# bglid/GTCRN-Micro

Hardware: AMD Instinct MI355X
Metric: 16 kHz frames/sec (STFT->mask->iSTFT) (higher is better)
Workload: dtype f32; 1 GPU; offline wave->wave, B=256 clips/GPU x 4 s @16 kHz (T=251 frames), fp32, shipped checkpoint weights; batch_per_gpu=256, parallelism=1 independent utterance shards, no data-path collective

## Files before the change

### gtcrn_micro_amd/csrc/api.cpp

```cpp
#include "../../include/gtcrn_micro_hip.h"

#include <hip/hip_runtime.h>

#include <cmath>
#include <cstdint>
#include <cstdio>
#include <cstring>
#include <mutex>
#include <string>
#include <vector>

#include "kernels.h"
#include "layout.h"
#include "pack.h"

namespace {

thread_local std::string g_err;

int fail(int code, const std::string& msg) {
    g_err = msg;
    return code;
}
int hip_fail(hipError_t e, const char* what) {
// ... 32 lines not shown
    float* d_pfq = nullptr;
    int* d_pi = nullptr;
    float* d_twid = nullptr;
    int* d_pref = nullptr;
    bool var_spans = true;
    int stream_form = 0;
    std::vector<int> h_pi;
    long cap_bt = 0;
    int last_B = 0, last_T = 0;
    float* d_en0 = nullptr;
    float* d_en[4] = {nullptr, nullptr, nullptr, nullptr};
    float* d_g1 = nullptr;
    float* d_g2 = nullptr;
    float* d_spec_a = nullptr;
    float* d_spec_b = nullptr;
    float* d_rate_a = nullptr;
    float* d_rate_b = nullptr;
    long cap_rate = 0;
    bool debug = false;
    bool debug_keep_fused = false;
    float* d_dbg = nullptr;
    long dbg_cap_bt = 0;
    unsigned long long* d_stamps = nullptr;
    int stamps_cap_b = 0;
    float** d_ptr8 = nullptr;
    bool last_quant = false;
    bool last_fused_stream = false;
    bool timing = false;
    int timing_only = -1;
    std::vector<Timing> timings;
    std::vector<Timing> ev_pool;
};

namespace {

void free_workspace(gtcrn_model* m) {
    float** bufs[] = {&m->d_en0, &m->d_en[0], &m->d_en[1], &m->d_en[2], &m->d_en[3], &m->d_g1, &m->d_g2,
                      &m->d_spec_a, &m->d_spec_b};
    for (float** p : bufs) {
        if (*p) (void)hipFree(*p);
        *p = nullptr;
    }
    m->cap_bt = 0;
}

int ensure_workspace(gtcrn_model* m, int B, int T, hipStream_t s) {
    const long bt = (long)B * T;
    if (bt > m->cap_bt) {
        hipStreamCaptureStatus cs = hipStreamCaptureStatusNone;
        if (hipStreamIsCapturing(s, &cs) == hipSuccess && cs != hipStreamCaptureStatusNone)
            return fail(GTCRN_ERR_STATE, "workspace too small during stream capture: call gtcrn_model_reserve first");
        HIP_TRY(hipDeviceSynchronize());
        free_workspace(m);
        HIP_TRY(hipMalloc(&m->d_en0, sizeof(float) * bt * 65 * 16));
        for (int i = 0; i < 4; ++i) HIP_TRY(hipMalloc(&m->d_en[i], sizeof(float) * bt * 528));
        HIP_TRY(hipMalloc(&m->d_g1, sizeof(float) * bt * 528));
        HIP_TRY(hipMalloc(&m->d_g2, sizeof(float) * bt * 528));
        HIP_TRY(hipMalloc(&m->d_spec_a, sizeof(float) * bt * 514));
        HIP_TRY(hipMalloc(&m->d_spec_b, sizeof(float) * bt * 514));
        m->cap_bt = bt;
    }
    if (m->debug && bt > m->dbg_cap_bt) {
        if (m->d_dbg) (void)hipFree(m->d_dbg);
        m->d_dbg = nullptr;
        HIP_TRY(hipMalloc(&m->d_dbg, sizeof(float) * bt * (3 * 528 + 65 * 16 + 2 * 129)));
        m->dbg_cap_bt = bt;
    }
    if (m->debug && B + 2048 > m->stamps_cap_b) {
        const int rows = B + 2048;
        if (m->d_stamps) (void)hipFree(m->d_stamps);
        m->d_stamps = nullptr;
        HIP_TRY(hipMalloc(&m->d_stamps, sizeof(unsigned long long) * 4 * rows * 16));
        HIP_TRY(hipMemset(m->d_stamps, 0, sizeof(unsigned long long) * 4 * rows * 16));
        m->stamps_cap_b = rows;
// ... 24 lines not shown
    void end() {
        if (!on) return;
        (void)hipEventRecord(m->timings.back().b, s);
    }
};

static bool stream_wide_pays(int B) {
    constexpr double WIDE_COST = 1.5;
    const int ws = gtk::stream_wide_streams();
    const long r4 = ((B + 3) / 4 + 255) / 256, r7 = ((B + ws - 1) / ws + 255) / 256;
    return (double)r7 * WIDE_COST < (double)r4;
}

int run_model(gtcrn_model* m, const float* spec_in, long isb, long isf, long ist, float* spec_out, long osb, long osf,
              long ost, int B, int T, float* state, hipStream_t s, const int* lens = nullptr,
              const gtk::Quant* q = nullptr, bool front_done = false) {
    Timer tm(m, s);
    const float* pf = q ? m->d_pfq : m->d_pf;
    const bool offline = !state;
    m->last_quant = q != nullptr;
    m->last_fused_stream = false;
    if (state && T == 1 && !q && (!m->debug || m->debug_keep_fused) && m->stream_form != 1 && gtk::stream_ms_usable(isb, osb)) {
        const bool wide = m->stream_form == 3 || (m->stream_form == 0 && stream_wide_pays(B));
        unsigned long long* stamps = (m->debug && m->d_stamps) ? m->d_stamps : nullptr;
        tm.begin(wide ? K_STREAM_WIDE : K_STREAM_MS);
        if (wide) LAUNCH_TRY(gtk::launch_stream_wide(spec_in, isb, isf, spec_out, osb, osf, B, pf, m->d_pi, state, stamps, s));
        else LAUNCH_TRY(gtk::launch_stream_ms(spec_in, isb, isf, spec_out, osb, osf, B, pf, m->d_pi, state, stamps, s));
        tm.end();
        m->last_fused_stream = true;
        m->last_B = B;
        m->last_T = T;
// ... 30 lines not shown
            LAUNCH_TRY(gtk::launch_gtcn(m->d_en[3], m->d_g1, pf + gtl::P_GTCN, B, T, state, gtk::ST_G1_H, nullptr,
                                        stp ? stp + sst : nullptr, s));
        tm.end();
        tm.begin(K_GTCN2);
        if (!state)
            LAUNCH_TRY(gtk::launch_gtcn_band(m->d_g1, m->d_g2, pf + gtl::P_GTCN + gtl::GTCN_SIZE, B, T, lens, m->d_en[3], s,
                                             q, pref));
        else
            LAUNCH_TRY(gtk::launch_gtcn(m->d_g1, m->d_g2, pf + gtl::P_GTCN + gtl::GTCN_SIZE, B, T, state, gtk::ST_G2_H,
                                        m->d_en[3], stp ? stp + 2 * sst : nullptr, s));
        tm.end();
    }
    tm.begin(K_DECODER);
    LAUNCH_TRY(gtk::launch_decoder(m->d_g2, m->d_en0, m->d_en[0], m->d_en[1], m->d_en[2], m->d_en[3], spec_in, isb, isf,
                                   ist, spec_out, osb, osf, ost, B, T, lens, pf, m->d_pi, state,
                                   m->debug && !q ? m->d_dbg : nullptr, stp ? stp + 3 * sst : nullptr, s, q, pref));
    tm.end();
    m->last_B = B;
    m->last_T = T;
    return 0;
}

int check_model(gtcrn_model* m) {
    if (!m || !m->d_pf) return fail(GTCRN_ERR_STATE, "invalid model handle");
    HIP_TRY(hipSetDevice(m->device));
    return 0;
}

int upload_params(gtcrn_model* m, const float* h_params, long n) {
    std::vector<float> F(gtl::P_FLOATS);
    std::vector<int> I(gtl::P_INTS);
// ... 230 lines not shown
    int rc = check_model(m);
    if (rc) return rc;
    if (!d_wave || !d_wave_out || !d_win) return fail(GTCRN_ERR_ARG, "null pointer");
    if (B < 1) return fail(GTCRN_ERR_ARG, "B must be >= 1");
    if (L < 257) return fail(GTCRN_ERR_ARG, "reflect padding needs L > 256 samples");
    hipStream_t s = (hipStream_t)stream;
    const int T = (int)gtcrn_num_frames(L);
    rc = ensure_workspace(m, B, T, s);
    if (rc) return rc;
    const long sb = (long)T * 514, sf = 2, st = 514;
    Timer tm(m, s);
    tm.begin(K_FRONT);
    LAUNCH_TRY(gtk::launch_front(d_wave, L, nullptr, 0, 0, 0, B, T, d_lengths, d_win, m->d_twid, q ? m->d_pfq : m->d_pf,
                                 m->d_pi, m->d_spec_a, m->d_en0, m->d_en[0], s, q));
    tm.end();
    rc = run_model(m, m->d_spec_a, sb, sf, st, m->d_spec_b, sb, sf, st, B, T, nullptr, s, d_lengths, q, true);
    if (rc) return rc;
    tm.begin(K_ISTFT);
    LAUNCH_TRY(gtk::launch_istft(m->d_spec_b, sb, sf, st, B, T, d_lengths, d_win, m->d_twid, d_wave_out, s));
    tm.end();
    return 0;
}

int gtcrn_forward_wave(gtcrn_model* m, const float* d_wave, float* d_wave_out, int B, long L, const float* d_win,
                       void* stream) {
    return forward_wave_impl(m, d_wave, d_wave_out, B, L, nullptr, d_win, stream);
}

int gtcrn_forward_wave_var(gtcrn_model* m, const float* d_wave, float* d_wave_out, int B, long Lmax,
                           const int* d_lengths, const float* d_win, void* stream) {
// ... 868 lines not shown
```

### gtcrn_micro_amd/csrc/kernels.h

```cpp
#pragma once
#include <hip/hip_runtime.h>

namespace gtk {

constexpr int TC = 16;
constexpr int NW = 11;
constexpr int NTHR = NW * 64;
constexpr int NT2 = TC * 33 / 16;
constexpr int TPW = NT2 / NW;
constexpr int SHORT_T = (NW * 16) / 33;
constexpr int SHORT_T2 = (2 * NW * 16) / 33;
static_assert(TC * 33 % 16 == 0, "chunk must be a whole number of tiles");
static_assert(NT2 % NW == 0, "tiles must divide evenly over the waves");

constexpr int FRAMES_PER_WAVE = 2;
constexpr int ISTFT_BLOCKS = 7;

constexpr int WS_RING = 0;
constexpr int WS_TAIL = 512;
constexpr int WS_CNT = 768;
constexpr int WS_FLOATS = 772;
constexpr int WS_CNT_MAX = 1 << 30;
constexpr int WAVE_FRAMES = 2;
static_assert(WS_FLOATS % 4 == 0, "16-byte aligned rows");
// ... 6 lines not shown
constexpr int ST_DEC_H = ST_G2_H + 30 * 33 * 16;
constexpr int ST_DEC_E = ST_DEC_H + 3 * 2 * 33 * 16;
constexpr int ST_FLOATS = ST_DEC_E + 48;

struct Quant {
    float in_step = 0.f;
    float out_step = 0.f;
};

int configure_kernels();
int launch_stft(const float* wave, int B, long L, int T, const int* lens, const float* win, const float* twid,
                float* spec, long sb, long sf, long st, float* frames, hipStream_t s);
int launch_pcm16_convert(const void* src, void* dst, long n, int dir, hipStream_t s);
int launch_istft(const float* spec, long sb, long sf, long st, int B, int T, const int* lens, const float* win,
                 const float* twid, float* wave, hipStream_t s);
template <typename S>
int launch_wave_analysis(const S* in, long in_stride, int N, int nhops, int r, bool flush, const float* wstate,
                         const float* win, const float* twid, float* spec, hipStream_t s);
template <typename S>
int launch_wave_synthesis(const float* spec, const S* in, long in_stride, S* out, long out_stride, int N, int nhops, int r,
                          bool flush, float* wstate, const float* win, const float* twid, hipStream_t s);
constexpr int RS_THREADS = 256;
constexpr int RS_TILE = 1024;
constexpr int RS_SPAN = 3328;
constexpr int RS_LDS_TAPS = 1024;
constexpr int RATE_SPAN = 1024;
long resample_tile_span(int up, int down, int ntp);
template <typename SI, typename SO>
int launch_resample(const SI* in, long in_stride, const int* lens, long L, SO* out, long out_stride, int B, int up, int down,
                    int half, int ntp, const float* taps, hipStream_t s);
// ... 20 lines not shown
int launch_encoder(const float* spec, long sb, long sf, long st, int B, int T, const int* lens, const float* PF,
                   const int* PI, float* en0, float* en1, float* en2, float* en3, float* en4, float* state,
                   unsigned long long* stamps, hipStream_t s, const Quant* q = nullptr, bool front_done = false,
                   const int* pref = nullptr);
int launch_front(const float* wave, long L, const float* spec_in, long isb, long isf, long ist, int B, int T,
                 const int* lens, const float* win, const float* twid, const float* PF, const int* PI, float* spec_out,
                 float* en0, float* en1p, hipStream_t s, const Quant* q = nullptr);
int launch_gtcn(const float* xin, float* xout, const float* P, int B, int T, float* state, int st_off,
                const float* addend, unsigned long long* stamps, hipStream_t s);
int launch_gtcn_ms(const float* xin, float* xout1, float* xout2, const float* P, int B, float* state, hipStream_t s);
int launch_gtcn_band(const float* xin, float* xout, const float* P, int B, int T, const int* lens, const float* addend,
                     hipStream_t s, const Quant* q = nullptr, const int* pref = nullptr);
int launch_decoder(const float* xg, const float* en0, const float* en1, const float* en2, const float* en3,
                   const float* en4, const float* spec, long sb, long sf, long st, float* out, long osb, long osf,
                   long ost, int B, int T, const int* lens, const float* PF, const int* PI, float* state, float* dbg,
                   unsigned long long* stamps, hipStream_t s, const Quant* q = nullptr, const int* pref = nullptr);
bool var_spans_usable(int B);
int launch_len_prefix(const int* lens, int B, int T, int* pref, hipStream_t s);
int launch_stream_ms(const float* spec, long sb, long sf, float* out, long osb, long osf, int B, const float* PF,
                     const int* PI, float* state, unsigned long long* stamps, hipStream_t s);
int launch_stream_wide(const float* spec, long sb, long sf, float* out, long osb, long osf, int B, const float* PF,
                       const int* PI, float* state, unsigned long long* stamps, hipStream_t s);
int stream_wide_streams();
bool stream_ms_usable(long sb, long osb);
int launch_state_convert(float* state, int N, float* conv, float* tra, float* const* tcn8, const int* PI, int dir,
                         hipStream_t s);
int launch_conv2d_causal(const float* x, const float* cache, const float* w, const float* bias, float* y,
                         float* cache_out, int B, int Cin, int Cout, int T, int F, int kt, int kf, int dt, int df,
                         int pf, int groups, int transposed, int Fout, hipStream_t s);
int launch_selftest(const float* A, const float* Bm, const float* C, float* D, hipStream_t s);
int launch_selftest_split3(const float* x, long n, float* planes, float* joined, const float* A, const float* Bm,
// ... 4 lines not shown
```

### gtcrn_micro_amd/csrc/kernels.hip

```cpp
#include <hip/hip_runtime.h>

#include <cstdint>
#include <cstdio>
#include <cstdlib>
#include <type_traits>

#include "kernels.h"
#include "layout.h"

using namespace gtl;

namespace gtk {

typedef float f32x4 __attribute__((ext_vector_type(4)));
typedef float f32x2 __attribute__((ext_vector_type(2)));

__device__ __forceinline__ f32x4 ld4(const float* p) { return *reinterpret_cast<const f32x4*>(p); }
__device__ __forceinline__ void st4(float* p, f32x4 v) { *reinterpret_cast<f32x4*>(p) = v; }
__device__ __forceinline__ void copy_params(float* dst, const float* src, int n, int tid, int nthr) {
    for (int i = 4 * tid; i < n; i += 4 * nthr) st4(dst + i, ld4(src + i));
}
__device__ __forceinline__ f32x4 splat(float v) { f32x4 r = {v, v, v, v}; return r; }
__device__ __forceinline__ void lds_dma_1k(const float* gsrc_lane, const float* lds_piece) {
    const unsigned lds_dst = (unsigned)(size_t)(__attribute__((address_space(3))) const void*)lds_piece;
// ... 93 lines not shown
}
template <bool Q>
__device__ __forceinline__ float rq1(float v) {
    if constexpr (Q) return (float)(_Float16)v;
    else return v;
}
template <bool Q>
__device__ __forceinline__ f32x4 rq(const f32x4 v) {
    if constexpr (Q) {
        const h16x4 h = to_h4(v);
        f32x4 r = {(float)h[0], (float)h[1], (float)h[2], (float)h[3]};
        return r;
    } else {
        return v;
    }
}
template <bool Q>
__device__ __forceinline__ f32x4 mm1(const f32x4 A, const f32x4 b, f32x4 acc) {
    if constexpr (Q) {
        return mfma_h(to_h4(A), to_h4(b), acc);
    } else {
#pragma unroll
        for (int s = 0; s < 4; ++s) acc = mfma(A[s], b[s], acc);
        return acc;
    }
}
template <int N, bool Q = false>
__device__ __forceinline__ void mm16(const f32x4 A, const f32x4 (&x)[N], f32x4 (&acc)[N]) {
    if constexpr (Q) {
        const h16x4 ah = to_h4(A);
// ... 262 lines not shown
                    *ok = make_float2(old.x + ck * (ze.x + r.x), old.y + (k == 0 ? 0.f : ck * (ze.y + r.y)));
                    if (k == 0) { const float2 o2 = *on; *on = make_float2(o2.x + (zk.x - zk.y) * (1.0f / 512.0f), o2.y); }
                } else {
                    *ok = make_float2(ze.x + r.x, ze.y + r.y);
                    if (k == 0)
                        *on = make_float2(zk.x - zk.y, 0.f);
                }
            }
        }
        wave_lds_sync();
#pragma unroll
        for (int q = 0; q < 4; ++q) cur[q] = nxt[q];
    }
}

__global__ __launch_bounds__(FFT_WAVES * 64) void k_istft(const float* __restrict__ spec, long sb, long sf, long st,
                                                         int B, int T, const int* __restrict__ lens,
                                                         const float* __restrict__ win,
                                                         const float2* __restrict__ twid, float* __restrict__ wave) {
    __shared__ float2 s_tw[256];
    __shared__ float2 s_tw512[256];
    __shared__ float s_win[512];
    __shared__ float2 s_fa[ISTFT_BLOCKS + 1][256];
    __shared__ float2 s_fb[FFT_WAVES][256];
    float (*s_fr)[512] = reinterpret_cast<float (*)[512]>(&s_fa[0][0]);
    static_assert(ISTFT_BLOCKS + 1 <= 2 * FFT_WAVES, "one buffer per frame of the two rounds");
    const int tid = threadIdx.x, lane = tid & 63, wv = tid >> 6;
    for (int i = tid; i < 256; i += FFT_WAVES * 64) { s_tw[i] = twid[i]; s_tw512[i] = twid[256 + i]; }
    for (int i = tid; i < 512; i += FFT_WAVES * 64) s_win[i] = win[i];
    __syncthreads();
    const int groups = (T - 1 + ISTFT_BLOCKS - 1) / ISTFT_BLOCKS;
    const int b = blockIdx.x / groups, grp = blockIdx.x - b * groups;
    const int nblk = lens ? (lens[b] >> 8) : T - 1;
    const int j0 = grp * ISTFT_BLOCKS;
    if (j0 >= nblk) return;
    const int nfr = min(ISTFT_BLOCKS, nblk - j0) + 1;
    constexpr int ROUNDS = (ISTFT_BLOCKS + 1 + FFT_WAVES - 1) / FFT_WAVES;
    auto fetch = [&](int it, float2 (&vk)[4], float2 (&vm)[4]) {
        const int fi = it * FFT_WAVES + wv;
        const int t = j0 + (fi < nfr ? fi : 0);
        const float* x = spec + (long)b * sb + (long)t * st;
#pragma unroll
        for (int q = 0; q < 4; ++q) {
            const int k = lane + 64 * q;
            vk[q] = *reinterpret_cast<const float2*>(x + (long)k * sf);
            vm[q] = *reinterpret_cast<const float2*>(x + (long)(256 - k) * sf);
        }
    };
    float2 ck[4], cm[4], nk[4], nm[4];
    fetch(0, ck, cm);
    for (int it = 0; it < ROUNDS; ++it) {
        const int fi = it * FFT_WAVES + wv;
        const bool live = fi < nfr;
        float2* A = s_fa[fi < ISTFT_BLOCKS + 1 ? fi : ISTFT_BLOCKS];
        float2* Bf = s_fb[wv];
        if (it + 1 < ROUNDS) fetch(it + 1, nk, nm);
#pragma unroll
        for (int q = 0; q < 4; ++q) {
            const int k = lane + 64 * q;
            float2 xk = ck[q];
            float2 xm = cm[q];
            xm.y = -xm.y;
            if (k == 0) { xk.y = 0.f; xm.y = 0.f; }
            const float2 xe = make_float2(0.5f * (xk.x + xm.x), 0.5f * (xk.y + xm.y));
            float2 w = s_tw512[k];
            w.y = -w.y;
            const float2 xo = cmul(make_float2(0.5f * (xk.x - xm.x), 0.5f * (xk.y - xm.y)), w);
            A[k] = make_float2(xe.x - xo.y, xe.y + xo.x);
        }
        wave_lds_sync();
        fft256<1>(A, Bf, s_tw, lane);
        if (live) {
#pragma unroll
            for (int q = 0; q < 4; ++q) {
                const int m = lane + 64 * q;
                const float2 z = A[m];
                s_fr[fi][2 * m] = (z.x * (1.0f / 256.0f)) * s_win[2 * m];
                s_fr[fi][2 * m + 1] = (z.y * (1.0f / 256.0f)) * s_win[2 * m + 1];
            }
        }
        wave_lds_sync();
#pragma unroll
        for (int q = 0; q < 4; ++q) { ck[q] = nk[q]; cm[q] = nm[q]; }
    }
    __syncthreads();
    float* o = wave + (long)b * 256 * (T - 1);
    for (int idx = tid; idx < (nfr - 1) * 256; idx += FFT_WAVES * 64) {
        const int jb = idx >> 8, i = idx & 255;
        const float acc = s_fr[jb][256 + i] + s_fr[jb + 1][i];
        const float env = s_win[256 + i] * s_win[256 + i] + s_win[i] * s_win[i];
        o[(long)(j0 + jb) * 256 + i] = env > 1e-11f ? acc / env : acc;
    }
}

template <typename S>
__device__ __forceinline__ float wave_ld(const S* p) {
    if constexpr (std::is_same<S, short>::value) return (float)*p * (1.0f / 32768.0f);
    else return *p;
}
template <typename S>
__device__ __forceinline__ void wave_st(S* p, float y) {
    if constexpr (std::is_same<S, short>::value) *p = (short)(int)fminf(fmaxf(__builtin_rintf(y * 32768.0f), -32768.0f), 32767.0f);
    else *p = y;
}

template <typename S, bool FLUSH>
__global__ __launch_bounds__(FFT_WAVES * 64) void k_wave_analysis(const S* __restrict__ in, long in_stride, int N,
// ... 1772 lines not shown
    static constexpr int PT = MS ? 35 : 41;
    static constexpr int S = A + RWI * PT * RS;
    static constexpr int ZSZ = RW * DEC_Z_ROW * DEC_ZS;
    static constexpr int M = A + ZSZ;
    static constexpr int MSZ = (2 * RW * F0 + 4 + 3) & ~3;
    static constexpr int AEND = (S + RW * 33 * RSS) > (M + MSZ) ? (S + RW * 33 * RSS) : (M + MSZ);
    static constexpr int BS = AEND;
    static constexpr int FLOATS = BS + NBINS * 4;
    static_assert(M % 4 == 0 && BS % 4 == 0 && D_BS_W % 4 == 0 && D_BS_TAB % 4 == 0 && S % 4 == 0 && DL_SIZE % 4 == 0, "16B carve");
    static_assert(FLOATS * 4 <= 160 * 1024, "decoder LDS budget");
    static_assert(DEC_SIZE % 4 == 0 && I % 4 == 0 && H % 4 == 0 && A % 4 == 0 && E % 4 == 0, "16B carve");
};
constexpr int DEC_LDS_FLOATS = DecLds<TC, 1, false>::FLOATS;
constexpr int DEC_MS_LDS_FLOATS = DecLds<MS_ROWS, MS_STREAMS, true>::FLOATS;

template <bool DBG, int TPW, bool MS, bool Q, bool SPANS = false>
__global__ __launch_bounds__(NTHR) void k_decoder(const float* __restrict__ xg, const float* __restrict__ en0,
                                                 const float* __restrict__ en1, const float* __restrict__ en2,
                                                 const float* __restrict__ en3, const float* __restrict__ en4,
                                                 const float* __restrict__ spec, long sb, long sf, long st,
                                                 float* __restrict__ out, long osb, long osf, long ost, int T,
                                                 const int* __restrict__ lens, int NB, float qin, float qout,
                                                 const float* __restrict__ PF, const int* __restrict__ PI,
                                                 float* __restrict__ state, float* __restrict__ dbg,
                                                 unsigned long long* __restrict__ stamps) {
    extern __shared__ __attribute__((aligned(16))) float smem[];
    STAMP_INIT(SS)
    constexpr int RW = MS ? MS_ROWS : TC;
    constexpr int NS = MS ? MS_STREAMS : 1;
    using LD = DecLds<RW, NS, MS>;
    float* sP = smem + LD::P;
    int* sI = reinterpret_cast<int*>(smem + LD::I);
    float* sH = smem + LD::H;
    float* sEH = smem + LD::EH;
    int* sTB = reinterpret_cast<int*>(smem + LD::TB);
    float* sG = smem + LD::G;
    constexpr int RS = LD::RS;
    float* sW = smem + LD::A;
    float* sS = smem + LD::S;
    float* sZ = smem + LD::A;
    constexpr int ZS = DEC_ZS;
    float* sM = smem + LD::M;
    float* sBS = smem + LD::BS;
    const Lane L = lane_info();
    const int tid = L.tid, n = L.n, g = L.g;
    const int Tstride = T;
    static_assert(!SPANS || (!MS && !Q), "time spans: offline fp32 form");
    SpanIter sit;
    #ifdef GT_EXP_SAMEUTT
    int s_b = blockIdx.x & 7, s_fb = 0, s_wlo = 0, s_nT = T;
#else
    int s_b = blockIdx.x, s_fb = 0, s_wlo = 0, s_nT = T;
#endif
    if constexpr (SPANS) {
        if (!span_begin(sit, blockIdx.x, gridDim.x, NB, T, lens)) return;
        span_next(sit, NB, Tstride, lens, HALO_BLOCKS, s_b, s_fb, s_wlo, s_nT);
    }
    int b = s_b;
    constexpr bool SPLIT = !Q && kSplitDense;
    constexpr bool HALFW = Q && !MS;
    constexpr int DN_PIECES = SPLIT ? DN16_SIZE / 256 : (HALFW ? DN16_CHUNKS : 9);
    auto dense_fetch = [&](int j) {
// ... 2 lines not shown
        asm volatile("" : "+v"(lz));
        for (int pi = L.wave; pi < DN_PIECES; pi += NW) {
            const float* gsrc = src + pi * 256 + 4 * lz;
            const unsigned lds_dst = (unsigned)(size_t)(__attribute__((address_space(3))) void*)(sP + DL_DN + pi * 256);
            unsigned keep;
            asm volatile("s_mov_b32 %0, m0\n\ts_mov_b32 m0, %2\n\ts_nop 0\n\tglobal_load_lds_dwordx4 %1, off\n\ts_mov_b32 m0, %0"
                         : "=&s"(keep)
                         : "v"(gsrc), "s"(lds_dst)
                         : "memory");
        }
    };
    dense_fetch(0);
    constexpr bool SPLIT3 = SPLIT && kSplitDe3;
    copy_dec_params<SPLIT3>(sP, PF, tid, NTHR);
    if (tid < 48) sI[tid] = PI[I_DEC_BLK + tid];
    for (int f = tid; f < NBINS; f += NTHR) st4(sBS + f * 4, ld4(PF + P_DEC + D_BS_TAB + f * 4));
    if (tid < 4) sM[2 * RW * F0 + tid] = 0.f;
    float* stb = state ? state + (long)b * NS * ST_FLOATS : nullptr;
    const int nlive = MS ? min(NS, NB - b * NS) : 1;
    int tbase = 0;
    if constexpr (MS) {
        rings_load_ms<NS, SPLIT ? RS_WIDE : 16>(sH, sEH, stb, ST_DEC_H, ST_DEC_E, nlive, tid);
        if (tid < 8) sTB[tid] = tid < nlive ? reinterpret_cast<const int*>(stb + (long)tid * ST_FLOATS)[0] : 0;
    } else {
        tbase = stb ? reinterpret_cast<const int*>(stb)[0] : 0;
        rings_load(sH, sEH, stb ? stb + ST_DEC_H : nullptr, stb ? stb + ST_DEC_E : nullptr, tbase, tid);
    }
    const Tiles<TPW> tt = make_tiles<TPW>(L);
    wg_barrier_vm();

    const long nbt = MS ? (long)gridDim.x * T : (long)NB * T;
    const float* const spec0 = spec;
// ... 123 lines not shown
        for (int i = 0; i < TPW; ++i) {
            if (g < 3) {
                st4(sZ + (tt.tl[i] * DEC_Z_ROW + 1 + 2 * tt.ff[i]) * ZS + 4 * g, ze[i]);
                if (tt.ff[i] < 32) st4(sZ + (tt.tl[i] * DEC_Z_ROW + 2 + 2 * tt.ff[i]) * ZS + 4 * g, zo[i]);
            }
        }
        {
            int tz = tid;
            asm volatile("" : "+v"(tz));
            if (tz < RW * 2 * 4 && (tz & 3) < 3) {
                float z = 0.f;
                asm volatile("" : "+v"(z));
                st4(sZ + ((tz >> 3) * DEC_Z_ROW + ((tz >> 2) & 1) * (DEC_Z_ROW - 1)) * ZS + 4 * (tz & 3), splat(z));
            }
        }
        float2 spv[MASK_ITEMS];
        {
            int tz = tid;
            asm volatile("" : "+v"(tz));
            int tq, f;
            spec_item_first(tz, t_fast, tq, f);
            const float* sbase = spec + (long)t0 * st;
#pragma unroll
            for (int q = 0; q < MASK_ITEMS; ++q) {
                const bool ok = tq < nfr && f < NBINS;
                spv[q] = *reinterpret_cast<const float2*>(sbase + (ok ? f * sf32 + tq * st32 : 0));
                spec_item_next(t_fast, tq, f);
            }
        }
        STAMP(SS, 15)
        wg_barrier();
        STAMP(SS, 12)
// ... 4 lines not shown
            for (int i = 0; i < TPW; ++i) xn[i] = ldx<Q>(xgn + (unsigned)((tt.pp(i) < npn ? tt.pp(i) : 0) * 16 + 4 * g));
        }
        {
            static_assert(4 * F0 <= NTHR && RW % 2 == 0, "two threads per (o, f'')");
            int tz = tid;
            asm volatile("" : "+v"(tz));
            if (tz < 4 * F0) {
                const int h = tz >= 2 * F0 ? 1 : 0, c = tz - h * 2 * F0, o = c >= F0 ? 1 : 0, fq = c - o * F0;
                const int par = fq & 1, m = fq >> 1;
                const float* zr = sZ + (h * DEC_Z_ROW + 1 + m) * ZS;
                const float* r1 = zr + ZS + o * 5 + par;
                const float* r2 = zr + o * 5 + 2 + par;
                const float* r3 = zr - ZS + (par ? 10 : o * 5 + 4);
                const float bias = sP[dl(D_DE4_B) + o];
                float* mo = sM + (o * RW + h) * F0 + fq;
#pragma unroll
                for (int j = 0; j < RW / 2; ++j) {
                    constexpr int ZF = 2 * DEC_Z_ROW * ZS;
                    const float sum = bias + r1[j * ZF] + r2[j * ZF] + r3[j * ZF];
                    mo[j * 2 * F0] = rq1<Q>(fast_tanh(sum));
                }
            }
        }
        wg_barrier();
        STAMP(SS, 13)
        if (DBG)
            for (int idx = tid; idx < 2 * nfr * F0; idx += NTHR) {
                const int fq = idx % F0, ot = idx / F0, o = ot >= nfr ? 1 : 0, tq = ot - o * nfr;
                if (t0 + tq >= wlo)
                    dbg[3 * nbt * 528 + nbt * F1 * 16 + (((long)b * 2 + o) * Tstride + (ob - (long)b * Tstride) + t0 + tq) * F0 + fq] =
                        sM[(o * RW + tq) * F0 + fq];
            }
        {
            int tz = tid;
            asm volatile("" : "+v"(tz));
            int tq, f;
            spec_item_first(tz, t_fast, tq, f);
            float* obase = out + (long)t0 * ost;
            constexpr int GRP = 3;
            static_assert(MASK_ITEMS % GRP == 0, "mask items come in groups of three");
#pragma unroll
            for (int q0 = 0; q0 < MASK_ITEMS; q0 += GRP) {
                bool ok[GRP], wr[GRP];
                int fo[GRP];
                const float* m0[GRP];
                f32x4 tb[GRP];
#pragma unroll
                for (int j = 0; j < GRP; ++j) {
// ... 1 lines not shown
                    wr[j] = ok[j] && t0 + tq >= wlo;
                    const int fc = ok[j] ? f : 0, tc = ok[j] ? tq : 0;
                    tb[j] = ld4(sBS + fc * 4);
                    m0[j] = sM + tc * F0;
                    fo[j] = f * osf32 + tq * ost32;
                    spec_item_next(t_fast, tq, f);
                }
                float a0[GRP], a1[GRP], b0[GRP], b1[GRP];
#pragma unroll
                for (int j = 0; j < GRP; ++j) {
                    const float* mp = m0[j] + __float_as_int(tb[j][0]);
                    a0[j] = mp[0]; a1[j] = mp[1]; b0[j] = mp[RW * F0]; b1[j] = mp[RW * F0 + 1];
                }
#pragma unroll
                for (int j = 0; j < GRP; ++j) {
                    const bool two = tb[j][2] != 0.f;
                    const float mr = rq1<Q>(tb[j][1] * a0[j] + (two ? tb[j][2] * a1[j] : 0.f));
                    const float mi = rq1<Q>(tb[j][1] * b0[j] + (two ? tb[j][2] * b1[j] : 0.f));
                    float re = spv[q0 + j].x, im = spv[q0 + j].y;
                    if constexpr (Q) {
                        if (qin > 0.f) {
                            re = fminf(fmaxf(rintf(re / qin), -128.f), 127.f) * qin;
                            im = fminf(fmaxf(rintf(im / qin), -128.f), 127.f) * qin;
                        }
                        re = rq1<Q>(re);
                        im = rq1<Q>(im);
                    }
                    float yr = rq1<Q>(re * mr - im * mi), yi = rq1<Q>(im * mr + re * mi);
                    if constexpr (Q) {
                        if (qout > 0.f) {
                            yr = fminf(fmaxf(rintf(yr / qout), -128.f), 127.f) * qout;
                            yi = fminf(fmaxf(rintf(yi / qout), -128.f), 127.f) * qout;
                        }
                    }
                    if (wr[j]) *reinterpret_cast<float2*>(obase + fo[j]) = make_float2(yr, yi);
                }
            }
        }
        wg_barrier();
        STAMP(SS, 14)
    }
    if constexpr (SPANS) {
        if (span_next(sit, NB, Tstride, lens, HALO_BLOCKS, s_b, s_fb, s_wlo, s_nT)) {
// ... 3 lines not shown
            goto segment_top;
        }
    }
    STAMP_OUT(SS, stamps)
    if (stb) {
        wg_barrier();
        if constexpr (MS) {
            rings_store_ms<NS, SPLIT ? RS_WIDE : 16>(sH, sEH, stb, ST_DEC_H, ST_DEC_E, nlive, tid);
            if (tid < nlive) reinterpret_cast<int*>(stb + (long)tid * ST_FLOATS)[0] = (sTB[tid] + 1) & 0xFFFF;
        } else {
            rings_store(sH, sEH, stb + ST_DEC_H, stb + ST_DEC_E, tbase + T, tid);
            if (tid == 0) reinterpret_cast<int*>(stb)[0] = (tbase + T) & 0xFFFF;
        }
    }
}

__device__ __forceinline__ void stagger_start(int unit) {
#ifndef GT_EXP_NOSTAGGER
    if (unit > 0 && blockIdx.x < 256) {
        const int ph = ((blockIdx.x >> 3) + 32 * (blockIdx.x & 7)) & ((unit >> 8) - 1);
        for (int i = 0; i < ph * (unit & 255); ++i) __builtin_amdgcn_s_sleep(8);
    }
#endif
}
struct SmLds {
    static constexpr int RW = MS_ROWS, NS = MS_STREAMS;
    static constexpr int PE = 0;
    static constexpr int PG = PE + ENC_SIZE;
    static constexpr int PD = PG + 2 * GTCN_SIZE;
    static constexpr int I = PD + DL_SIZE;
// ... 1383 lines not shown
                       (const int*)nullptr, win,
                       reinterpret_cast<const float2*>(twid), gspec, sb, sf, st, (float*)nullptr);
    GT_LAUNCH_CHECK();
    return 0;
}

int launch_istft(const float* spec, long sb, long sf, long st, int B, int T, const int* lens, const float* win,
                 const float* twid, float* wave, hipStream_t s) {
    const int groups = (T - 1 + ISTFT_BLOCKS - 1) / ISTFT_BLOCKS;
    hipLaunchKernelGGL(k_istft, dim3(B * groups), dim3(FFT_WAVES * 64), 0, s, spec, sb, sf, st, B, T, lens, win,
                       reinterpret_cast<const float2*>(twid), wave);
    GT_LAUNCH_CHECK();
    return 0;
}

int configure_kernels() {
    hipError_t e;
    const void* enc[] = {reinterpret_cast<const void*>(k_encoder<TPW, false, false, false, true>),
                         reinterpret_cast<const void*>(k_encoder<TPW, false, false, true>),
                         reinterpret_cast<const void*>(k_encoder<1, false, false, true>),
                         reinterpret_cast<const void*>(k_encoder<2, false, false, true>),
                         reinterpret_cast<const void*>(k_encoder<TPW, false, false, false>),
                         reinterpret_cast<const void*>(k_encoder<1, false, false, false>),
                         reinterpret_cast<const void*>(k_encoder<2, false, false, false>),
                         reinterpret_cast<const void*>(k_encoder<TPW, false, true, false>)};
    const void* fr[] = {reinterpret_cast<const void*>(k_front<true, false>), reinterpret_cast<const void*>(k_front<false, false>),
                        reinterpret_cast<const void*>(k_front<true, true>), reinterpret_cast<const void*>(k_front<false, true>)};
    for (const void* f : fr) {
        e = hipFuncSetAttribute(f, hipFuncAttributeMaxDynamicSharedMemorySize, FR_LDS_FLOATS * 4);
        if (e != hipSuccess) return (int)e;
// ... 26 lines not shown
    if (e != hipSuccess) return (int)e;
    e = hipFuncSetAttribute(reinterpret_cast<const void*>(k_gtcn_band<true>), hipFuncAttributeMaxDynamicSharedMemorySize,
                            GB_LDS_FLOATS * 4);
    if (e != hipSuccess) return (int)e;
    e = hipFuncSetAttribute(reinterpret_cast<const void*>(k_gtcn_band<false, true>), hipFuncAttributeMaxDynamicSharedMemorySize,
                            GB_LDS_FLOATS * 4);
    if (e != hipSuccess) return (int)e;
    const void* dec[] = {reinterpret_cast<const void*>(k_decoder<false, TPW, false, false, true>),
                         reinterpret_cast<const void*>(k_decoder<true, TPW, false, false, true>),
                         reinterpret_cast<const void*>(k_decoder<false, TPW, false, false>),
                         reinterpret_cast<const void*>(k_decoder<true, TPW, false, false>),
                         reinterpret_cast<const void*>(k_decoder<false, 1, false, false>),
                         reinterpret_cast<const void*>(k_decoder<true, 1, false, false>),
                         reinterpret_cast<const void*>(k_decoder<false, 2, false, false>),
                         reinterpret_cast<const void*>(k_decoder<true, 2, false, false>),
                         reinterpret_cast<const void*>(k_decoder<false, TPW, false, true>)};
    for (const void* f : dec) {
        e = hipFuncSetAttribute(f, hipFuncAttributeMaxDynamicSharedMemorySize, DEC_LDS_FLOATS * 4);
        if (e != hipSuccess) return (int)e;
    }
    return 0;
}

static bool use_multi_stream(int T, const float* state, long sb) {
    return state != nullptr && T == 1 && (MS_ROWS - 1) * (sb < 0 ? -sb : sb) < (1L << 31);
}

int launch_front(const float* wave, long L, const float* spec_in, long isb, long isf, long ist, int B, int T,
                 const int* lens, const float* win, const float* twid, const float* PF, const int* PI, float* spec_out,
                 float* en0, float* en1p, hipStream_t s, const Quant* q) {
    const long wgs = ((long)B * T + FR_WAVES - 1) / FR_WAVES;
// ... 100 lines not shown
    if (pl.nA)
        hipLaunchKernelGGL(k_gtcn_band<false>, dim3(pl.nA), dim3(NTHR), GB_LDS_FLOATS * 4, s, xin, xout, P, pl.nA, T, lens,
                           addend);
    if (pl.nwgB) {
        const long o = (long)pl.nA * T * 528;
        hipLaunchKernelGGL((k_gtcn_band<false, true>), dim3(pl.nwgB), dim3(NTHR), GB_LDS_FLOATS * 4, s, xin + o, xout + o, P,
                           B - pl.nA, T, lens, addend ? addend + o : nullptr);
    }
    GT_LAUNCH_CHECK();
    return 0;
}

int launch_decoder(const float* xg, const float* en0, const float* en1, const float* en2, const float* en3,
                   const float* en4, const float* spec, long sb, long sf, long st, float* out, long osb, long osf,
                   long ost, int B, int T, const int* lens, const float* PF, const int* PI, float* state, float* dbg,
                   unsigned long long* stamps, hipStream_t s, const Quant* q, const int* pref) {
    if (pref && !state && !q) {
        const int nwg = var_span_workgroups(B);
        if (dbg)
            hipLaunchKernelGGL((k_decoder<true, TPW, false, false, true>), dim3(nwg), dim3(NTHR), DEC_LDS_FLOATS * 4, s, xg, en0,
                               en1, en2, en3, en4, spec, sb, sf, st, out, osb, osf, ost, T, pref, B, 0.f, 0.f, PF, PI, state, dbg,
                               stamps);
        else
            hipLaunchKernelGGL((k_decoder<false, TPW, false, false, true>), dim3(nwg), dim3(NTHR), DEC_LDS_FLOATS * 4, s, xg, en0,
                               en1, en2, en3, en4, spec, sb, sf, st, out, osb, osf, ost, T, pref, B, 0.f, 0.f, PF, PI, state, dbg,
                               stamps);
        GT_LAUNCH_CHECK();
        return 0;
    }
    SpanPlan pl = span_plan(B, T, HALO_BLOCKS, !state && !q && lens == nullptr);
    if (dbg && pl.nA && pl.nwgB) {
// ... 373 lines not shown
```

Baseline: 58.18 million frames/s.

## Hand off raw mask to iSTFT and apply band gain there

In the offline wave-to-wave path the decoder now writes only the raw tanh mask (258 floats per frame) to a new buffer, skipping the band-split gain and complex multiply on the spectrum. The iSTFT kernel reads the mask alongside the input spectrum, expands it through the band table in LDS and applies the complex ratio mask before the inverse FFT. The intent is to drop the decoder's spectrum read, its 514-float-per-frame masked spectrum write, and one decoder LDS barrier, at the cost of extra registers and LDS traffic in the iSTFT, now pinned to an occupancy of 5 waves per EU.

New measurement: 58.15 million frames/s. Within noise of the previous version (-0.1%).

```diff
diff --git a/gtcrn_micro_amd/csrc/api.cpp b/gtcrn_micro_amd/csrc/api.cpp
--- a/gtcrn_micro_amd/csrc/api.cpp
+++ b/gtcrn_micro_amd/csrc/api.cpp
@@ -70,6 +70,7 @@
     float* d_g2 = nullptr;
     float* d_spec_a = nullptr;
     float* d_spec_b = nullptr;
+    float* d_mask = nullptr;
     float* d_rate_a = nullptr;
     float* d_rate_b = nullptr;
     long cap_rate = 0;
@@ -92,7 +93,7 @@
 
 void free_workspace(gtcrn_model* m) {
     float** bufs[] = {&m->d_en0, &m->d_en[0], &m->d_en[1], &m->d_en[2], &m->d_en[3], &m->d_g1, &m->d_g2,
-                      &m->d_spec_a, &m->d_spec_b};
+                      &m->d_spec_a, &m->d_spec_b, &m->d_mask};
     for (float** p : bufs) {
         if (*p) (void)hipFree(*p);
         *p = nullptr;
@@ -114,6 +115,7 @@
         HIP_TRY(hipMalloc(&m->d_g2, sizeof(float) * bt * 528));
         HIP_TRY(hipMalloc(&m->d_spec_a, sizeof(float) * bt * 514));
         HIP_TRY(hipMalloc(&m->d_spec_b, sizeof(float) * bt * 514));
+        HIP_TRY(hipMalloc(&m->d_mask, sizeof(float) * bt * gtk::MASK_ROW));
         m->cap_bt = bt;
     }
     if (m->debug && bt > m->dbg_cap_bt) {
@@ -168,7 +170,7 @@
 
 int run_model(gtcrn_model* m, const float* spec_in, long isb, long isf, long ist, float* spec_out, long osb, long osf,
               long ost, int B, int T, float* state, hipStream_t s, const int* lens = nullptr,
-              const gtk::Quant* q = nullptr, bool front_done = false) {
+              const gtk::Quant* q = nullptr, bool front_done = false, bool mask_out = false) {
     Timer tm(m, s);
     const float* pf = q ? m->d_pfq : m->d_pf;
     const bool offline = !state;
@@ -229,7 +231,7 @@
     tm.begin(K_DECODER);
     LAUNCH_TRY(gtk::launch_decoder(m->d_g2, m->d_en0, m->d_en[0], m->d_en[1], m->d_en[2], m->d_en[3], spec_in, isb, isf,
                                    ist, spec_out, osb, osf, ost, B, T, lens, pf, m->d_pi, state,
-                                   m->debug && !q ? m->d_dbg : nullptr, stp ? stp + 3 * sst : nullptr, s, q, pref));
+                                   m->debug && !q ? m->d_dbg : nullptr, stp ? stp + 3 * sst : nullptr, s, q, pref, mask_out));
     tm.end();
     m->last_B = B;
     m->last_T = T;
@@ -490,6 +492,17 @@
     LAUNCH_TRY(gtk::launch_front(d_wave, L, nullptr, 0, 0, 0, B, T, d_lengths, d_win, m->d_twid, q ? m->d_pfq : m->d_pf,
                                  m->d_pi, m->d_spec_a, m->d_en0, m->d_en[0], s, q));
     tm.end();
+    const bool mask_out = gtk::mask_handoff_enabled() && !q && !m->debug;
+    if (mask_out) {
+        const long mr = gtk::MASK_ROW;
+        rc = run_model(m, m->d_spec_a, sb, sf, st, m->d_mask, (long)T * mr, 1, mr, B, T, nullptr, s, d_lengths, q, true, true);
+        if (rc) return rc;
+        tm.begin(K_ISTFT);
+        LAUNCH_TRY(gtk::launch_istft_mask(m->d_spec_a, sb, sf, st, m->d_mask, m->d_pf, B, T, d_lengths, d_win, m->d_twid,
+                                          d_wave_out, s));
+        tm.end();
+        return 0;
+    }
     rc = run_model(m, m->d_spec_a, sb, sf, st, m->d_spec_b, sb, sf, st, B, T, nullptr, s, d_lengths, q, true);
     if (rc) return rc;
     tm.begin(K_ISTFT);
diff --git a/gtcrn_micro_amd/csrc/kernels.h b/gtcrn_micro_amd/csrc/kernels.h
--- a/gtcrn_micro_amd/csrc/kernels.h
+++ b/gtcrn_micro_amd/csrc/kernels.h
@@ -44,6 +44,10 @@
 int launch_pcm16_convert(const void* src, void* dst, long n, int dir, hipStream_t s);
 int launch_istft(const float* spec, long sb, long sf, long st, int B, int T, const int* lens, const float* win,
                  const float* twid, float* wave, hipStream_t s);
+constexpr int MASK_ROW = 258;
+bool mask_handoff_enabled();
+int launch_istft_mask(const float* spec, long sb, long sf, long st, const float* mask, const float* PF, int B, int T,
+                      const int* lens, const float* win, const float* twid, float* wave, hipStream_t s);
 template <typename S>
 int launch_wave_analysis(const S* in, long in_stride, int N, int nhops, int r, bool flush, const float* wstate,
                          const float* win, const float* twid, float* spec, hipStream_t s);
@@ -94,7 +98,8 @@
 int launch_decoder(const float* xg, const float* en0, const float* en1, const float* en2, const float* en3,
                    const float* en4, const float* spec, long sb, long sf, long st, float* out, long osb, long osf,
                    long ost, int B, int T, const int* lens, const float* PF, const int* PI, float* state, float* dbg,
-                   unsigned long long* stamps, hipStream_t s, const Quant* q = nullptr, const int* pref = nullptr);
+                   unsigned long long* stamps, hipStream_t s, const Quant* q = nullptr, const int* pref = nullptr,
+                   bool mask_out = false);
 bool var_spans_usable(int B);
 int launch_len_prefix(const int* lens, int B, int T, int* pref, hipStream_t s);
 int launch_stream_ms(const float* spec, long sb, long sf, float* out, long osb, long osf, int B, const float* PF,
diff --git a/gtcrn_micro_amd/csrc/kernels.hip b/gtcrn_micro_amd/csrc/kernels.hip
--- a/gtcrn_micro_amd/csrc/kernels.hip
+++ b/gtcrn_micro_amd/csrc/kernels.hip
@@ -131,6 +131,17 @@
     } else {
         return v;
     }
+}
+template <bool Q>
+__device__ __forceinline__ void bs_gain(float w0, float w1, float a0, float a1, float b0, float b1, float& mr, float& mi) {
+    const bool two = w1 != 0.f;
+    mr = rq1<Q>(w0 * a0 + (two ? w1 * a1 : 0.f));
+    mi = rq1<Q>(w0 * b0 + (two ? w1 * b1 : 0.f));
+}
+template <bool Q>
+__device__ __forceinline__ void crm_apply(float re, float im, float mr, float mi, float& yr, float& yi) {
+    yr = rq1<Q>(re * mr - im * mi);
+    yi = rq1<Q>(im * mr + re * mi);
 }
 template <bool Q>
 __device__ __forceinline__ f32x4 mm1(const f32x4 A, const f32x4 b, f32x4 acc) {
@@ -423,10 +434,11 @@
     }
 }
 
-__global__ __launch_bounds__(FFT_WAVES * 64) void k_istft(const float* __restrict__ spec, long sb, long sf, long st,
-                                                         int B, int T, const int* __restrict__ lens,
-                                                         const float* __restrict__ win,
-                                                         const float2* __restrict__ twid, float* __restrict__ wave) {
+template <bool MIN>
+__device__ __forceinline__ void istft_body(const float* __restrict__ spec, long sb, long sf, long st, int B, int T,
+                                           const int* __restrict__ lens, const float* __restrict__ win,
+                                           const float2* __restrict__ twid, float* __restrict__ wave,
+                                           const float* __restrict__ mask, const float* __restrict__ bstab) {
     __shared__ float2 s_tw[256];
     __shared__ float2 s_tw512[256];
     __shared__ float s_win[512];
@@ -445,7 +457,8 @@
     if (j0 >= nblk) return;
     const int nfr = min(ISTFT_BLOCKS, nblk - j0) + 1;
     constexpr int ROUNDS = (ISTFT_BLOCKS + 1 + FFT_WAVES - 1) / FFT_WAVES;
-    auto fetch = [&](int it, float2 (&vk)[4], float2 (&vm)[4]) {
+    constexpr int NMR = MIN ? 5 : 1;
+    auto fetch = [&](int it, float2 (&vk)[4], float2 (&vm)[4], float (&vr)[NMR]) {
         const int fi = it * FFT_WAVES + wv;
         const int t = j0 + (fi < nfr ? fi : 0);
         const float* x = spec + (long)b * sb + (long)t * st;
@@ -455,15 +468,52 @@
             vk[q] = *reinterpret_cast<const float2*>(x + (long)k * sf);
             vm[q] = *reinterpret_cast<const float2*>(x + (long)(256 - k) * sf);
         }
+        if constexpr (MIN) {
+            const float* mrow = mask + ((long)b * T + t) * MASK_ROW;
+#pragma unroll
+            for (int q = 0; q < 4; ++q) vr[q] = mrow[lane + 64 * q];
+            vr[4] = mrow[256 + (lane & 1)];
+        }
     };
+    int bi[MIN ? 8 : 1];
+    float bw0[MIN ? 8 : 1], bw1[MIN ? 8 : 1];
+    if constexpr (MIN) {
+#pragma unroll
+        for (int q = 0; q < 8; ++q) {
+            const int f = q < 4 ? lane + 64 * q : 256 - (lane + 64 * (q - 4));
+            const f32x4 row = ld4(bstab + f * 4);
+            bi[q] = __float_as_int(row[0]); bw0[q] = row[1]; bw1[q] = row[2];
+        }
+    }
     float2 ck[4], cm[4], nk[4], nm[4];
-    fetch(0, ck, cm);
+    float cr[NMR], nr[NMR];
+    fetch(0, ck, cm, cr);
     for (int it = 0; it < ROUNDS; ++it) {
         const int fi = it * FFT_WAVES + wv;
         const bool live = fi < nfr;
         float2* A = s_fa[fi < ISTFT_BLOCKS + 1 ? fi : ISTFT_BLOCKS];
         float2* Bf = s_fb[wv];
-        if (it + 1 < ROUNDS) fetch(it + 1, nk, nm);
+        if (it + 1 < ROUNDS) fetch(it + 1, nk, nm, nr);
+        if constexpr (MIN) {
+            float* mb = reinterpret_cast<float*>(Bf);
+#pragma unroll
+            for (int q = 0; q < 4; ++q) mb[lane + 64 * q] = cr[q];
+            if (lane < 2) mb[256 + lane] = cr[4];
+            wave_lds_sync();
+            float a0[8], a1[8], b0[8], b1[8];
+#pragma unroll
+            for (int q = 0; q < 8; ++q) {
+                const float* mp = mb + bi[q];
+                a0[q] = mp[0]; a1[q] = mp[1]; b0[q] = mp[F0]; b1[q] = mp[F0 + 1];
+            }
+#pragma unroll
+            for (int q = 0; q < 8; ++q) {
+                float mr, mi;
+                bs_gain<false>(bw0[q], bw1[q], a0[q], a1[q], b0[q], b1[q], mr, mi);
+                float2& v = q < 4 ? ck[q] : cm[q - 4];
+                crm_apply<false>(v.x, v.y, mr, mi, v.x, v.y);
+            }
+        }
 #pragma unroll
         for (int q = 0; q < 4; ++q) {
             const int k = lane + 64 * q;
@@ -491,6 +541,8 @@
         wave_lds_sync();
 #pragma unroll
         for (int q = 0; q < 4; ++q) { ck[q] = nk[q]; cm[q] = nm[q]; }
+#pragma unroll
+        for (int q = 0; q < NMR; ++q) cr[q] = nr[q];
     }
     __syncthreads();
     float* o = wave + (long)b * 256 * (T - 1);
@@ -500,6 +552,20 @@
         const float env = s_win[256 + i] * s_win[256 + i] + s_win[i] * s_win[i];
         o[(long)(j0 + jb) * 256 + i] = env > 1e-11f ? acc / env : acc;
     }
+}
+__global__ __launch_bounds__(FFT_WAVES * 64) void k_istft(const float* __restrict__ spec, long sb, long sf, long st,
+                                                         int B, int T, const int* __restrict__ lens,
+                                                         const float* __restrict__ win,
+                                                         const float2* __restrict__ twid, float* __restrict__ wave) {
+    istft_body<false>(spec, sb, sf, st, B, T, lens, win, twid, wave, nullptr, nullptr);
+}
+__global__ __launch_bounds__(FFT_WAVES * 64) __attribute__((amdgpu_waves_per_eu(5, 5))) void k_istft_mask(const float* __restrict__ spec, long sb, long sf, long st,
+                                                              int B, int T, const int* __restrict__ lens,
+                                                              const float* __restrict__ win,
+                                                              const float2* __restrict__ twid, float* __restrict__ wave,
+                                                              const float* __restrict__ mask,
+                                                              const float* __restrict__ bstab) {
+    istft_body<true>(spec, sb, sf, st, B, T, lens, win, twid, wave, mask, bstab);
 }
 
 template <typename S>
@@ -2302,16 +2368,16 @@
 constexpr int DEC_LDS_FLOATS = DecLds<TC, 1, false>::FLOATS;
 constexpr int DEC_MS_LDS_FLOATS = DecLds<MS_ROWS, MS_STREAMS, true>::FLOATS;
 
-template <bool DBG, int TPW, bool MS, bool Q, bool SPANS = false>
-__global__ __launch_bounds__(NTHR) void k_decoder(const float* __restrict__ xg, const float* __restrict__ en0,
-                                                 const float* __restrict__ en1, const float* __restrict__ en2,
-                                                 const float* __restrict__ en3, const float* __restrict__ en4,
-                                                 const float* __restrict__ spec, long sb, long sf, long st,
-                                                 float* __restrict__ out, long osb, long osf, long ost, int T,
-                                                 const int* __restrict__ lens, int NB, float qin, float qout,
-                                                 const float* __restrict__ PF, const int* __restrict__ PI,
-                                                 float* __restrict__ state, float* __restrict__ dbg,
-                                                 unsigned long long* __restrict__ stamps) {
+template <bool DBG, int TPW, bool MS, bool Q, bool SPANS, bool MOUT>
+__device__ __forceinline__ void decoder_body(const float* __restrict__ xg, const float* __restrict__ en0,
+                                             const float* __restrict__ en1, const float* __restrict__ en2,
+                                             const float* __restrict__ en3, const float* __restrict__ en4,
+                                             const float* __restrict__ spec, long sb, long sf, long st,
+                                             float* __restrict__ out, long osb, long osf, long ost, int T,
+                                             const int* __restrict__ lens, int NB, float qin, float qout,
+                                             const float* __restrict__ PF, const int* __restrict__ PI,
+                                             float* __restrict__ state, float* __restrict__ dbg,
+                                             unsigned long long* __restrict__ stamps) {
     extern __shared__ __attribute__((aligned(16))) float smem[];
     STAMP_INIT(SS)
     constexpr int RW = MS ? MS_ROWS : TC;
@@ -2334,6 +2400,9 @@
     const int tid = L.tid, n = L.n, g = L.g;
     const int Tstride = T;
     static_assert(!SPANS || (!MS && !Q), "time spans: offline fp32 form");
+    static_assert(!MOUT || (!MS && !Q), "mask-out: offline fp32 form");
+    static_assert(MASK_ROW == 2 * F0, "mask hand-off row");
+    constexpr bool KEEP_M = !MOUT || DBG;
     SpanIter sit;
     #ifdef GT_EXP_SAMEUTT
     int s_b = blockIdx.x & 7, s_fb = 0, s_wlo = 0, s_nT = T;
@@ -2366,8 +2435,8 @@
     constexpr bool SPLIT3 = SPLIT && kSplitDe3;
     copy_dec_params<SPLIT3>(sP, PF, tid, NTHR);
     if (tid < 48) sI[tid] = PI[I_DEC_BLK + tid];
-    for (int f = tid; f < NBINS; f += NTHR) st4(sBS + f * 4, ld4(PF + P_DEC + D_BS_TAB + f * 4));
-    if (tid < 4) sM[2 * RW * F0 + tid] = 0.f;
+    if constexpr (!MOUT) for (int f = tid; f < NBINS; f += NTHR) st4(sBS + f * 4, ld4(PF + P_DEC + D_BS_TAB + f * 4));
+    if (KEEP_M && tid < 4) sM[2 * RW * F0 + tid] = 0.f;
     float* stb = state ? state + (long)b * NS * ST_FLOATS : nullptr;
     const int nlive = MS ? min(NS, NB - b * NS) : 1;
     int tbase = 0;
@@ -2521,8 +2590,8 @@
                 st4(sZ + ((tz >> 3) * DEC_Z_ROW + ((tz >> 2) & 1) * (DEC_Z_ROW - 1)) * ZS + 4 * (tz & 3), splat(z));
             }
         }
-        float2 spv[MASK_ITEMS];
-        {
+        float2 spv[MOUT ? 1 : MASK_ITEMS];
+        if constexpr (!MOUT) {
             int tz = tid;
             asm volatile("" : "+v"(tz));
             int tq, f;
@@ -2557,15 +2626,22 @@
                 const float* r3 = zr - ZS + (par ? 10 : o * 5 + 4);
                 const float bias = sP[dl(D_DE4_B) + o];
                 float* mo = sM + (o * RW + h) * F0 + fq;
+                float* mg = MOUT ? out + (long)t0 * ost : nullptr;
+                const int mgo = h * MASK_ROW + o * F0 + fq;
 #pragma unroll
                 for (int j = 0; j < RW / 2; ++j) {
                     constexpr int ZF = 2 * DEC_Z_ROW * ZS;
                     const float sum = bias + r1[j * ZF] + r2[j * ZF] + r3[j * ZF];
-                    mo[j * 2 * F0] = rq1<Q>(fast_tanh(sum));
+                    const float mv = rq1<Q>(fast_tanh(sum));
+                    if constexpr (KEEP_M) mo[j * 2 * F0] = mv;
+                    if constexpr (MOUT) {
+                        const int tq = h + 2 * j;
+                        if (tq < nfr && t0 + tq >= wlo) __builtin_nontemporal_store(mv, mg + mgo + j * 2 * MASK_ROW);
+                    }
                 }
             }
         }
-        wg_barrier();
+        if constexpr (KEEP_M) wg_barrier();
         STAMP(SS, 13)
         if (DBG)
             for (int idx = tid; idx < 2 * nfr * F0; idx += NTHR) {
@@ -2574,7 +2650,7 @@
                     dbg[3 * nbt * 528 + nbt * F1 * 16 + (((long)b * 2 + o) * Tstride + (ob - (long)b * Tstride) + t0 + tq) * F0 + fq] =
                         sM[(o * RW + tq) * F0 + fq];
             }
-        {
+        if constexpr (!MOUT) {
             int tz = tid;
             asm volatile("" : "+v"(tz));
             int tq, f;
@@ -2606,9 +2682,8 @@
                 }
 #pragma unroll
                 for (int j = 0; j < GRP; ++j) {
-                    const bool two = tb[j][2] != 0.f;
-                    const float mr = rq1<Q>(tb[j][1] * a0[j] + (two ? tb[j][2] * a1[j] : 0.f));
-                    const float mi = rq1<Q>(tb[j][1] * b0[j] + (two ? tb[j][2] * b1[j] : 0.f));
+                    float mr, mi;
+                    bs_gain<Q>(tb[j][1], tb[j][2], a0[j], a1[j], b0[j], b1[j], mr, mi);
                     float re = spv[q0 + j].x, im = spv[q0 + j].y;
                     if constexpr (Q) {
                         if (qin > 0.f) {
@@ -2618,7 +2693,8 @@
                         re = rq1<Q>(re);
                         im = rq1<Q>(im);
                     }
-                    float yr = rq1<Q>(re * mr - im * mi), yi = rq1<Q>(im * mr + re * mi);
+                    float yr, yi;
+                    crm_apply<Q>(re, im, mr, mi, yr, yi);
                     if constexpr (Q) {
                         if (qout > 0.f) {
                             yr = fminf(fmaxf(rintf(yr / qout), -128.f), 127.f) * qout;
@@ -2652,6 +2728,25 @@
         }
     }
 }
+#define GT_DEC_PARAMS                                                                                                 \
+    const float *__restrict__ xg, const float *__restrict__ en0, const float *__restrict__ en1,                      \
+        const float *__restrict__ en2, const float *__restrict__ en3, const float *__restrict__ en4,                 \
+        const float *__restrict__ spec, long sb, long sf, long st, float *__restrict__ out, long osb, long osf,      \
+        long ost, int T, const int *__restrict__ lens, int NB, float qin, float qout, const float *__restrict__ PF,  \
+        const int *__restrict__ PI, float *__restrict__ state, float *__restrict__ dbg,                              \
+        unsigned long long *__restrict__ stamps
+#define GT_DEC_ARGS                                                                                                   \
+    xg, en0, en1, en2, en3, en4, spec, sb, sf, st, out, osb, osf, ost, T, lens, NB, qin, qout, PF, PI, state, dbg, stamps
+template <bool DBG, int TPW, bool MS, bool Q, bool SPANS = false>
+__global__ __launch_bounds__(NTHR) void k_decoder(GT_DEC_PARAMS) {
+    decoder_body<DBG, TPW, MS, Q, SPANS, false>(GT_DEC_ARGS);
+}
+template <int TPW, bool SPANS>
+__global__ __launch_bounds__(NTHR) void k_decoder_mout(GT_DEC_PARAMS) {
+    decoder_body<false, TPW, false, false, SPANS, true>(GT_DEC_ARGS);
+}
+#undef GT_DEC_PARAMS
+#undef GT_DEC_ARGS
 
 __device__ __forceinline__ void stagger_start(int unit) {
 #ifndef GT_EXP_NOSTAGGER
@@ -4065,6 +4160,23 @@
     return 0;
 }
 
+bool mask_handoff_enabled() {
+#ifdef GT_MASK_IN_DECODER
+    return false;
+#else
+    return true;
+#endif
+}
+
+int launch_istft_mask(const float* spec, long sb, long sf, long st, const float* mask, const float* PF, int B, int T,
+                      const int* lens, const float* win, const float* twid, float* wave, hipStream_t s) {
+    const int groups = (T - 1 + ISTFT_BLOCKS - 1) / ISTFT_BLOCKS;
+    hipLaunchKernelGGL(k_istft_mask, dim3(B * groups), dim3(FFT_WAVES * 64), 0, s, spec, sb, sf, st, B, T, lens, win,
+                       reinterpret_cast<const float2*>(twid), wave, mask, PF + P_DEC + D_BS_TAB);
+    GT_LAUNCH_CHECK();
+    return 0;
+}
+
 int configure_kernels() {
     hipError_t e;
     const void* enc[] = {reinterpret_cast<const void*>(k_encoder<TPW, false, false, false, true>),
@@ -4121,7 +4233,11 @@
                          reinterpret_cast<const void*>(k_decoder<true, 1, false, false>),
                          reinterpret_cast<const void*>(k_decoder<false, 2, false, false>),
                          reinterpret_cast<const void*>(k_decoder<true, 2, false, false>),
-                         reinterpret_cast<const void*>(k_decoder<false, TPW, false, true>)};
+                         reinterpret_cast<const void*>(k_decoder<false, TPW, false, true>),
+                         reinterpret_cast<const void*>(k_decoder_mout<TPW, true>),
+                         reinterpret_cast<const void*>(k_decoder_mout<TPW, false>),
+                         reinterpret_cast<const void*>(k_decoder_mout<1, false>),
+                         reinterpret_cast<const void*>(k_decoder_mout<2, false>)};
     for (const void* f : dec) {
         e = hipFuncSetAttribute(f, hipFuncAttributeMaxDynamicSharedMemorySize, DEC_LDS_FLOATS * 4);
         if (e != hipSuccess) return (int)e;
@@ -4252,7 +4368,37 @@
 int launch_decoder(const float* xg, const float* en0, const float* en1, const float* en2, const float* en3,
                    const float* en4, const float* spec, long sb, long sf, long st, float* out, long osb, long osf,
                    long ost, int B, int T, const int* lens, const float* PF, const int* PI, float* state, float* dbg,
-                   unsigned long long* stamps, hipStream_t s, const Quant* q, const int* pref) {
+                   unsigned long long* stamps, hipStream_t s, const Quant* q, const int* pref, bool mask_out) {
+    if (mask_out) {
+        if (state || q || dbg || ost != MASK_ROW) return (int)hipErrorInvalidValue;
+#define GT_DEC_MOUT(TPWV, SPV, GRID, ...)                                                                          \
+    hipLaunchKernelGGL((k_decoder_mout<TPWV, SPV>), dim3(GRID), dim3(NTHR), DEC_LDS_FLOATS * 4, s, __VA_ARGS__)
+        const SpanPlan pl = span_plan(B, T, HALO_BLOCKS, lens == nullptr);
+        if (pref) {
+            GT_DEC_MOUT(TPW, true, var_span_workgroups(B), xg, en0, en1, en2, en3, en4, spec, sb, sf, st, out, osb, osf, ost, T,
+                        pref, B, 0.f, 0.f, PF, PI, state, dbg, stamps);
+        } else if (pl.nwgB) {
+            if (pl.nA)
+                GT_DEC_MOUT(TPW, false, pl.nA, xg, en0, en1, en2, en3, en4, spec, sb, sf, st, out, osb, osf, ost, T, lens,
+                            pl.nA, 0.f, 0.f, PF, PI, state, dbg, stamps);
+            const long o = (long)pl.nA * T * 528, o0 = (long)pl.nA * T * (F1 * 16);
+            GT_DEC_MOUT(TPW, true, pl.nwgB, xg + o, en0 + o0, en1 + o, en2 + o, en3 + o, en4 + o, spec + (long)pl.nA * sb, sb,
+                        sf, st, out + (long)pl.nA * osb, osb, osf, ost, T, lens, B - pl.nA, 0.f, 0.f, PF, PI, state, dbg,
+                        stamps ? stamps + (long)pl.nA * 16 : nullptr);
+        } else if (T <= SHORT_T) {
+            GT_DEC_MOUT(1, false, B, xg, en0, en1, en2, en3, en4, spec, sb, sf, st, out, osb, osf, ost, T, lens, B, 0.f, 0.f,
+                        PF, PI, state, dbg, stamps);
+        } else if (T <= SHORT_T2) {
+            GT_DEC_MOUT(2, false, B, xg, en0, en1, en2, en3, en4, spec, sb, sf, st, out, osb, osf, ost, T, lens, B, 0.f, 0.f,
+                        PF, PI, state, dbg, stamps);
+        } else {
+            GT_DEC_MOUT(TPW, false, B, xg, en0, en1, en2, en3, en4, spec, sb, sf, st, out, osb, osf, ost, T, lens, B, 0.f,
+                        0.f, PF, PI, state, dbg, stamps);
+        }
+#undef GT_DEC_MOUT
+        GT_LAUNCH_CHECK();
+        return 0;
+    }
     if (pref && !state && !q) {
         const int nwg = var_span_workgroups(B);
         if (dbg)
```
